# jcfaracco/xpysom-dask

Measured on AMD Instinct MI355X. Metric: samples/sec/epoch, higher is better.
Workload: dtype f16

## Files before the change

xpysom_dask_amd/_lib.py:

```python
import ctypes as C
import importlib.util
import os

HERE = os.path.dirname(os.path.abspath(__file__))
LIB_PATH = os.environ.get("SOM_LIB_PATH") or os.path.join(HERE, "libsomhip.so")

SOM_DIST = {"euclidean": 0, "euclidean_no_opt": 1, "cosine": 2, "manhattan": 3, "manhattan_no_opt": 3,
            "norm_p": 4, "norm_p_no_opt": 5}
SOM_NEIGH = {"gaussian": 0, "mexican_hat": 1, "bubble": 2, "triangle": 3}
SOM_PREC = {"f32": 0, "bf16": 1, "f16": 3, "exact": 5}
SOM_TOPO = {"rectangular": 0, "hexagonal": 1}
SOM_BMU_ACTIVATION, SOM_BMU_QUANTIZATION = 0, 1
SOM_KERNELS = {"bmu": 0, "segsum": 1, "kron": 2, "merge": 3, "prep": 4, "screen": 5}


class SomConfig(C.Structure):
    _fields_ = [("x", C.c_int32), ("y", C.c_int32), ("input_len", C.c_int32),
                ("distance", C.c_int32), ("neighborhood", C.c_int32),
                ("compact_support", C.c_int32), ("precision", C.c_int32), ("device", C.c_int32),
                ("std_coeff", C.c_double), ("stream", C.c_void_p),
                ("topology", C.c_int32), ("norm_p", C.c_int32), ("norm_p_real", C.c_double)]


_F = C.POINTER(C.c_float)
# ... 24 lines not shown
    "som_comm_init": (C.c_int, [_H, C.c_int32, C.c_int32, C.c_void_p]),
    "som_epoch_allreduce": (C.c_int, [_H]),
    "som_comm_destroy": (C.c_int, [_H]),
    "som_pinned_alloc": (C.c_int, [C.c_uint64, C.POINTER(C.c_void_p)]),
    "som_pinned_free": (C.c_int, [C.c_void_p]),
    "som_stream_begin": (C.c_int, [_H]),
    "som_stream_rows": (C.c_int, [_H, _F, C.c_int64]),
    "som_stream_end": (C.c_int, [_H, C.c_double, C.c_double, C.c_int]),
    "som_accum_device_ptr": (C.c_int, [_H, C.POINTER(C.c_void_p), C.POINTER(C.c_int64)]),
    "som_get_stream": (C.c_int, [_H, C.POINTER(C.c_void_p)]),
    "som_epoch_fetch": (C.c_int, [_H, _F, _F, _I]),
    "som_epoch_accumulate_forced": (C.c_int, [_H, _I, C.c_double, C.c_double, C.c_int]),
    "som_bmu": (C.c_int, [_H, _F, C.c_int64, C.c_int32, _I]),
    "som_bmu_device": (C.c_int, [_H, C.c_void_p, C.c_int64, C.c_int32, _I]),
    "som_bmu_top2": (C.c_int, [_H, _F, C.c_int64, _I, _I]),
    "som_bmu_top2_device": (C.c_int, [_H, C.c_void_p, C.c_int64, _I, _I]),
    "som_bmu_f64": (C.c_int, [_H, C.POINTER(C.c_double), C.c_int64, _I]),
    "som_distance_matrix": (C.c_int, [_H, _F, C.c_int64, C.c_int32, _F]),
    "som_quantization_error": (C.c_int, [_H, _F, C.c_int64, C.POINTER(C.c_double)]),
    "som_quantization_error_device": (C.c_int, [_H, C.c_void_p, C.c_int64, C.POINTER(C.c_double)]),
    "som_set_verify": (C.c_int, [_H, C.c_int32]),
    "som_verify_stats": (C.c_int, [_H, C.POINTER(C.c_int64), C.POINTER(C.c_int64)]),
    "som_debug_corrupt_operands": (C.c_int, [_H, C.c_int32]),
    "som_debug_mfma16": (C.c_int, [_H, C.c_void_p, C.c_void_p, _F, _F, C.c_int32]),
    "som_debug_stamps": (C.c_int, [_H, C.c_int64, C.c_void_p]),
    "som_debug_device_bytes": (C.c_int, [C.POINTER(C.c_int64)]),
    "som_debug_qe_stats": (C.c_int, [_H, C.POINTER(C.c_int64), C.POINTER(C.c_int64)]),
    "som_policy_eval": (C.c_int, [C.c_int32, C.POINTER(C.c_double), C.POINTER(C.c_double), C.POINTER(C.c_int32)]),
    "som_policy_replay": (C.c_int, [C.c_int32, C.POINTER(C.c_double), C.POINTER(C.c_double)]),
    "som_patch_order": (C.c_int, [C.c_int32, C.c_int32, _I]),
    "som_exact_stats": (C.c_int, [_H, C.POINTER(C.c_int64), C.POINTER(C.c_int64), C.POINTER(C.c_int64)]),
    "som_exact_top2_stats": (C.c_int, [_H, C.POINTER(C.c_int64), C.POINTER(C.c_int64)]),
    "som_exact_skip_stats": (C.c_int, [_H, C.POINTER(C.c_int64), C.POINTER(C.c_int64)]),
    "som_exact_resident_stats": (C.c_int, [_H, C.POINTER(C.c_int64), C.POINTER(C.c_int64)]),
    "som_exact_scout_stats": (C.c_int, [_H, C.POINTER(C.c_int64), C.POINTER(C.c_int64)]),
    "som_exact_refine_stats": (C.c_int, [_H, C.POINTER(C.c_int64), C.POINTER(C.c_int64)]),
    "som_exact_last_counts": (C.c_int, [_H, _I, C.c_int64]),
    "som_sync": (C.c_int, [_H]),
    "som_profile_enable": (C.c_int, [_H, C.c_int32]),
    "som_profile_get": (C.c_int, [_H, C.c_int32, C.POINTER(C.c_double), C.POINTER(C.c_int64)]),
    "som_profile_reset": (C.c_int, [_H]),
}

_lib = None


# ... 50 lines not shown
```

xpysom_dask_amd/csrc/bmu_bf16_k16.hpp:

```cpp
#pragma once
#include "bmu_bf16.hpp"

namespace somhip {

constexpr int K16_T = 4;
constexpr int K16_STAGE_UNITS = 16 * K16_T;
constexpr int K16_SB = 4;
constexpr int K16_NW = 4;
constexpr int K16_WG_SAMPLES = K16_NW * 16 * K16_SB;

__host__ __device__ constexpr int k16_stage_bytes(int ks32) { return (K16_T * ks32 + 1) * 1024; }

template <int KS32, class EL = Bf16>
__global__ __launch_bounds__(256) void prep_w_bf16_k16_kernel(const float* __restrict__ W, int K, int D,
                                                              char* __restrict__ Wst, int n_stages,
                                                              const float* __restrict__ unit_wsq,
                                                              const float* __restrict__ scale_max2 = nullptr) {
    using E = typename EL::T;
    using bf16x8 = typename V8<E>::t;
    long id = (long)blockIdx.x * 256 + threadIdx.x;
    long total = (long)n_stages * K16_T * KS32 * 64;
    if (id >= total) return;
    int lane = id & 63;
    long t = id >> 6;
    int ks = t % KS32; t /= KS32;
    int t16 = t % K16_T;
    long stage = t / K16_T;
    long u = stage * K16_STAGE_UNITS + t16 * 16 + (lane & 15);
    int k0 = ks * 32 + (lane >> 4) * 8;
    float scale = 1.0f;
    if (unit_wsq != nullptr && u < K) { float q = unit_wsq[u]; scale = q > 0.0f ? 1.0f / __builtin_sqrtf(q) : 0.0f; }
    if (scale_max2 != nullptr) scale = ex_scale(*scale_max2);
    bf16x8 v;
#pragma unroll
    for (int j = 0; j < 8; ++j) {
        float f = (u < K && k0 + j < D) ? W[u * D + k0 + j] * scale : 0.0f;
        v[j] = cvt<E>(-f);
    }
    *(bf16x8*)(Wst + stage * k16_stage_bytes(KS32) + ((long)(t16 * KS32 + ks) * 64 + lane) * 16) = v;
}

template <int KS32, class EL = Bf16>
__global__ __launch_bounds__(256) void prep_w_exact_k16_kernel(const float* __restrict__ W, int K, int D,
                                                               char* __restrict__ Wst, int n_stages,
                                                               const float* __restrict__ scale_max2,
                                                               float* __restrict__ werr2, char* __restrict__ Wst_lo = nullptr) {
    using E = typename EL::T;
    using bf16x8 = typename V8<E>::t;
    const int lane = threadIdx.x & 63;
    const long tile = (long)blockIdx.x * 4 + (threadIdx.x >> 6);
    if (tile >= (long)n_stages * K16_T) return;
    const long stage = tile / K16_T;
    const int t16 = (int)(tile - stage * K16_T);
    const long u = stage * K16_STAGE_UNITS + t16 * 16 + (lane & 15);
    const float scale = ex_scale(*scale_max2);
    float er = 0.0f;
#pragma unroll
    for (int ks = 0; ks < KS32; ++ks) {
        const int k0 = ks * 32 + (lane >> 4) * 8;
        bf16x8 v, vl;
#pragma unroll
        for (int j = 0; j < 8; ++j) {
            const float f = (u < K && k0 + j < D) ? W[u * D + k0 + j] * scale : 0.0f;
            const E hb = cvt<E>(-f);
            v[j] = hb;
            const float e = half_operand_error(-f, (float)hb);
            er = __builtin_fmaf(e, e, er);
            const float r = ((-f) - (float)hb) * 2048.0f;
            vl[j] = cvt<E>(r == r && __builtin_fabsf(r) < 3.0e38f ? r : 0.0f);
        }
        *(bf16x8*)(Wst + stage * k16_stage_bytes(KS32) + ((long)(t16 * KS32 + ks) * 64 + lane) * 16) = v;
        if (Wst_lo != nullptr) *(bf16x8*)(Wst_lo + stage * k16_stage_bytes(KS32) + ((long)(t16 * KS32 + ks) * 64 + lane) * 16) = vl;
// ... 417 lines not shown
```

xpysom_dask_amd/csrc/bmu_f32.hpp:

```cpp
#pragma once
#include "som_common.hpp"

namespace somhip {

constexpr int F32_SB = 128;
constexpr int F32_UB = 128;
constexpr int F32_KC = 32;

enum { SCORE_EUCLID_PART = 0, SCORE_EUCLID_SQRT = 1, SCORE_COSINE = 2, SCORE_EUCLID_SQ = 3 };

template <int MODE>
__device__ __forceinline__ float score_f32(float cross, float wsq, float xsq) {
    if (MODE == SCORE_EUCLID_PART) {
        return __builtin_fmaf(-2.0f, cross, wsq);
    } else if (MODE == SCORE_EUCLID_SQ) {
        return __builtin_fmaf(-2.0f, cross, wsq) + xsq;
    } else if (MODE == SCORE_EUCLID_SQRT) {
        float t = __builtin_fmaf(-2.0f, cross, wsq) + xsq;
        return nan_to_num_f32(__builtin_sqrtf(t));
    } else {
        float den = __builtin_sqrtf(xsq * wsq);
        return 1.0f - nan_to_num_f32(cross / den);
    }
}
// ... 76 lines not shown
        if (kc == 0 && tid < F32_UB) wq[tid] = (u0 + tid < K) ? wsq[u0 + tid] : 0.0f;
        __syncthreads();
        const float* xrow = Xs + (wave * 32 + col) * xstride + half;
        const float* wrow = Ws + col * (F32_KC + 1) + half;
#pragma unroll
        for (int k = 0; k < F32_KC; k += 2) {
            float b = xrow[k];
#pragma unroll
            for (int rb = 0; rb < 4; ++rb)
                acc[rb] = __builtin_amdgcn_mfma_f32_32x32x2f32(wrow[rb * 32 * (F32_KC + 1) + k], b, acc[rb], 0, 0, 0);
        }
    }
    if (my_sample < N) {
#pragma unroll
        for (int rb = 0; rb < 4; ++rb)
#pragma unroll
            for (int r = 0; r < 16; ++r) {
                int row = rb * 32 + mfma32_row(r, half);
                if (u0 + row < K) out[my_sample * K + u0 + row] = score_f32<MODE>(acc[rb][r], wq[row], xs);
            }
    }
}

__device__ float np_pairwise_sq_sum(const float* __restrict__ a, int n) {
    if (n < 8) {
        float res = 0.0f;
        for (int i = 0; i < n; ++i) res = __fadd_rn(res, __fmul_rn(a[i], a[i]));
        return res;
    }
    if (n <= 128) {
        float r[8];
#pragma unroll
        for (int j = 0; j < 8; ++j) r[j] = __fmul_rn(a[j], a[j]);
        int i = 8;
        for (; i < n - (n % 8); i += 8) {
#pragma unroll
            for (int j = 0; j < 8; ++j) r[j] = __fadd_rn(r[j], __fmul_rn(a[i + j], a[i + j]));
        }
        float res = __fadd_rn(__fadd_rn(__fadd_rn(r[0], r[1]), __fadd_rn(r[2], r[3])),
                              __fadd_rn(__fadd_rn(r[4], r[5]), __fadd_rn(r[6], r[7])));
        for (; i < n; ++i) res = __fadd_rn(res, __fmul_rn(a[i], a[i]));
        return res;
    }
    int n2 = n / 2;
    n2 -= n2 % 8;
    return __fadd_rn(np_pairwise_sq_sum(a, n2), np_pairwise_sq_sum(a + n2, n - n2));
}

__global__ __launch_bounds__(256) void row_sq_f32_kernel(const float* __restrict__ A, long rows, int D,
                                                         float* __restrict__ out, float* __restrict__ out_p = nullptr,
                                                         const int* __restrict__ inv = nullptr) {
    long row = (long)blockIdx.x * 256 + threadIdx.x;
    if (row >= rows) return;
    const float q = np_pairwise_sq_sum(A + row * (long)D, D);
    out[row] = q;
    if (out_p != nullptr) {
        out_p[inv[row]] = q;
    }
}

}
```

xpysom_dask_amd/csrc/exact_host.hpp:

```cpp

struct PassCtr {
    int* base; int n_groups;
    int* gcount() const { return base; }
    int* gstart() const { return base + n_groups; }
    PassCounters* tail() const { return (PassCounters*)(gstart() + n_groups); }
    RowNeed* row_need() const { return (RowNeed*)base; }
    size_t bytes() const { return 2 * (size_t)n_groups * sizeof(int) + sizeof(PassCounters); }
};
inline PassCtr pass_ctr(const som_handle* h) { return PassCtr{h->ex.ctr, (int)cdiv(h->K, EX_GROUP)}; }

constexpr double EX_KAPPA = 6.0;
ExactBound exact_bound(const som_handle* h) {
    const double u = std::ldexp(1.0, -24);
    const double Dl = h->wide ? 32.0 * h->ft_kchunks : 8.0 * h->fr_kg;
    const double n_mfma = h->wide ? h->n_kchunks : h->ks32;
    const double gamma = Dl * u / (1.0 - Dl * u);
    const double slop = 1.01;
    ExactBound eb{};
    eb.cB = (float)(slop * 2.0 * (EX_KAPPA * n_mfma + 1.0) * std::ldexp(1.0, -23));
    eb.cM = (float)(slop * 2.0);
    if (h->cfg.distance == SOM_DIST_COSINE) {
        eb.cA = (float)(slop * 2.0 * (gamma + 57.0 * u));
        eb.cW = 0.0f;
        eb.unit = 1;
// ... 244 lines not shown
        if (int rc = ex.tq.alloc(h, (size_t)stride)) return rc;
    if (int rc = ex.need.alloc(h, (size_t)tiles * ex.cen[0].n_cstages)) return rc;
    if (int rc = ex.need2.alloc(h, (size_t)tiles * ex.cen[1].n_cstages)) return rc;
    if (int rc = ex.glist.alloc(h, (size_t)tiles * n_groups)) return rc;
    if (int rc = ex.gcnt.alloc(h, (size_t)tiles)) return rc;
    if (int rc = ex.tile_counts.alloc(h, (size_t)tiles)) return rc;
    if (int rc = ex.tlist.alloc(h, (size_t)tiles * n_groups * K16_T)) return rc;
    if (int rc = ex.tcnt.alloc(h, (size_t)tiles)) return rc;
    ex.item_slots = (int)resident_slots(h, 8);
    if (int rc = ex.items.alloc(h, (size_t)(5 * tiles + 4 * ex.item_slots + 16))) return rc;
    if (int rc = ex.sk_tmp.alloc(h, radix_scratch_ints(stride))) return rc;
    ex.sk_stride = stride;
    return 0;
}

template <class E>
int exact_skip_centroids(som_handle* h, const float* xmax2) {
    auto& ex = h->ex;
    const float* Wsrc = h->ex_patch ? h->Wp : h->W;
    const int n_groups = (int)cdiv(h->K, EX_GROUP);
    auto& c0 = ex.cen[0];
    auto& c1 = ex.cen[1];
    const CentroidLevel l1{c0.Cc, c0.rg, c0.csq, c0.cmax2, c0.n_slots}, l2{c1.Cc, c1.rg, c1.csq, c1.cmax2, c1.n_slots};
    exact_centroids_kernel<<<dim3((unsigned)(cdiv(n_groups, 4) * 4)), dim3(512), 0, h->stream>>>(Wsrc, h->K, h->D, n_groups, l1, l2, h->wmax2);
    const int nst2 = ex.lp.level2 ? c1.n_cstages : 0;
    char* plain = ex.lp.scout ? c0.Cst_plain : nullptr;
    const dim3 tgrid((unsigned)cdiv((long)(c0.n_cstages + nst2) * K16_T, 4)), block(256);
    switch (h->ks32) {
#define SOM_CIMG_CASE(k) case k: exact_centroid_image_kernel<k, E><<<tgrid, block, 0, h->stream>>>(l1, c0.Cst, c0.n_cstages, l2, c1.Cst, nst2, h->D, xmax2, h->wmax2, plain); break;
    SOM_CIMG_CASE(1) SOM_CIMG_CASE(2) SOM_CIMG_CASE(3) SOM_CIMG_CASE(4)
#undef SOM_CIMG_CASE
    default: return fail(h, "exact: block skipping supports input_len <= 128");
    }
    HIPCHK(h, hipGetLastError());
    return 0;
}

int exact_skip_sortkeys(som_handle* h, som_handle::ExactScratch::SortedRows& sr, long s0, long n, const int* prev, const int* scout_g) {
    auto& ex = h->ex;
    const int n_groups = (int)cdiv(h->K, EX_GROUP);
    if (scout_g != nullptr)
        exact_groupkey_kernel<<<dim3((unsigned)cdiv(n, 256)), dim3(256), 0, h->stream>>>(scout_g, n, n_groups, ex.sk_keys, ex.sk_vals);
    else
        exact_sortkey_kernel<<<dim3((unsigned)cdiv(n, 256)), dim3(256), 0, h->stream>>>(prev, h->ex_inv, n, h->K, ex.sk_keys, ex.sk_vals);
    int bits = 1;
    while ((1L << bits) < n_groups) ++bits;
    return radix_sort_rows(h, ex.sk_keys, n, bits, ex.sk_keys2, sr.order + s0, ex.sk_tmp);
// ... 597 lines not shown
```

xpysom_dask_amd/csrc/exact_skip.hpp:

```cpp
#pragma once
#include "bmu_bf16_k16.hpp"

namespace somhip {

constexpr int SK_TILE = K16_WG_SAMPLES;
static_assert(K16_STAGE_UNITS == 64 && K16_T == 4, "block skipping: a stage of the resident screen is one 64-unit group of four 16-unit tiles");

struct CentroidLevel { float* C; float* rg; float* csq; float* cmax2; int n_slots; };
__global__ __launch_bounds__(512) void exact_centroids_kernel(const float* __restrict__ W, int K, int D, int n_groups,
                                                              CentroidLevel l1, CentroidLevel l2, const float* __restrict__ wmax2) {
    __shared__ float qsum[4][128];
    __shared__ float part[2][64][2];
    __shared__ float csq_s[2][5];
    const int g = blockIdx.x, tid = threadIdx.x, lane = tid & 63;
    const int d = tid & 127, q = tid >> 7, fh = (tid >> 6) & 1;
    const long u0 = (long)g * 64 + 16 * q;
    const int cnt = (int)max(0L, min(64L, (long)K - (long)g * 64));
    const int cb = max(0, min(16, cnt - 16 * q));
    if (g == 0 && tid == 0) { l1.cmax2[0] = *wmax2; l1.cmax2[1] = 0.0f; l2.cmax2[0] = *wmax2; l2.cmax2[1] = 0.0f; }
    float w[16];
#pragma unroll
    for (int k = 0; k < 16; ++k) w[k] = (d < D && k < cb) ? W[(u0 + k) * D + d] : 0.0f;
    float sum = 0.0f;
#pragma unroll
    for (int k = 0; k < 16; ++k) sum += w[k];
    qsum[q][d] = sum;
    __syncthreads();
    const float cs = cb > 0 ? sum / (float)cb : 0.0f;
    const float cg = cnt > 0 ? ((qsum[0][d] + qsum[1][d]) + (qsum[2][d] + qsum[3][d])) / (float)cnt : 0.0f;
    if (d < D) {
        if (q == 0 && g < l1.n_slots) l1.C[(long)g * D + d] = cg;
        const int j = 16 * (g >> 2) + 4 * (g & 3) + q;
        if (j < l2.n_slots) l2.C[(long)j * D + d] = cs;
    }
    {
        const float a = wave_sum(cs * cs);
        if (lane == 0) csq_s[fh][1 + q] = a;
        if (q == 0) { const float bq = wave_sum(cg * cg); if (lane == 0) csq_s[fh][0] = bq; }
    }
#pragma unroll
    for (int k = 0; k < 16; ++k) {
        if (k < cb) {
            const float dg = w[k] - cg, ds = w[k] - cs;
            const float qg = wave_sum(d < D ? dg * dg : 0.0f);
            const float qs = wave_sum(d < D ? ds * ds : 0.0f);
            if (lane == 0) { part[fh][16 * q + k][0] = qg; part[fh][16 * q + k][1] = qs; }
        }
    }
    __syncthreads();
    if (tid < 5) {
        const int b = tid - 1;
        const int k0 = tid == 0 ? 0 : 16 * b, k1 = tid == 0 ? cnt : min(cnt, 16 * b + 16);
        float m = 0.0f;
        for (int k = k0; k < k1; ++k) {
            const float d2 = part[0][k][tid == 0 ? 0 : 1] + part[1][k][tid == 0 ? 0 : 1];
            m = (d2 > m || !(d2 == d2)) ? d2 : m;
        }
        const float r = k1 > k0 ? __builtin_sqrtf(m) * (1.0f + 1.0f / 512.0f) + 1.0e-30f : -1.0f;
        const float sq = csq_s[0][tid] + csq_s[1][tid];
        if (tid == 0) { if (g < l1.n_slots) { l1.rg[g] = r; l1.csq[g] = sq; } }
        else {
            const int j = 16 * (g >> 2) + 4 * (g & 3) + b;
            if (j < l2.n_slots) { l2.rg[j] = r; l2.csq[j] = sq; }
        }
    }
}

__global__ __launch_bounds__(256) void exact_sortkey_kernel(const int* __restrict__ prev, const int* __restrict__ inv, long n,
                                                            int K, int* __restrict__ keys, int* __restrict__ vals) {
    const long i = (long)blockIdx.x * 256 + threadIdx.x;
    if (i >= n) return;
    int u = prev[i];
    u = u < 0 ? 0 : u >= K ? K - 1 : u;
    keys[i] = (inv != nullptr ? inv[u] : u) >> 6;
    vals[i] = (int)i;
}

__global__ __launch_bounds__(256) void exact_lastpos_kernel(const int* __restrict__ prev, const int* __restrict__ order,
                                                            const int* __restrict__ inv, long n, int K, int* __restrict__ lastpos) {
    const long p = (long)blockIdx.x * 256 + threadIdx.x;
    if (p >= n) return;
    int u = prev[order[p]];
    u = u < 0 ? 0 : u >= K ? K - 1 : u;
    lastpos[p] = inv != nullptr ? inv[u] : u;
}

template <class EL>
// ... 648 lines not shown
```

xpysom_dask_amd/csrc/somhip.hip:

```cpp
#include <hip/hip_runtime.h>

#include <cstring>

#include <dlfcn.h>

#include <cmath>
#include <cstdio>
#include <cstdlib>
#include <algorithm>
#include <atomic>
#include <cstring>
#include <string>
#include <utility>
#include <vector>

#include "../../include/somhip.h"
#include "../../include/somhip_test.h"
#include "bmu_bf16_k16.hpp"
#include "bmu_bf16_tiled.hpp"
#include "bmu_bf16_wide.hpp"
#include "bmu_exact.hpp"
#include "exact_skip.hpp"
#include "exact_policy.hpp"
#include "exact_skip_wide.hpp"
// ... 88 lines not shown
        DevBuf<float> fbX;
        PassCounters* pass_host = nullptr;
        hipEvent_t fb_ready = nullptr;
        int64_t rows_total = 0, rows_fallback = 0, chunks = 0;
        int64_t blocks_run = 0, blocks_total = 0;
        long pass_rows_override = 0;
        long hook_refuse_above = 0, hook_pairs = 0; bool hook_refuse_skip = false;
        long stride_cap = 0;
        long pairs = 64;
        int skip_mode = 1;
        policy::PlanState plan;
        policy::LaunchPlan lp;
        bool sub_blocks = true;
        struct SortedRows {
            long cap = 0;
            DevBuf<int> order;
            DevBuf<__bf16> Xb_s;
            DevBuf<__bf16> Xl_s;
            bool xl_filled = false;
            DevBuf<float> Xf_s, xsq_s, xerr_s, seed_s, sU_s;
            DevBuf<int> lastpos_s;
        } srt[2];
        bool cen_ready = false;
        long sk_stride = 0;
        int res_every = 0;
        DevBuf<int> sk_keys, sk_keys2, sk_vals;
        DevBuf<int> sk_tmp;
        bool refine_on = true;
        int grid_mult = 2;
        bool scout_on = true;
        DevBuf<int> scout_g;
        DevBuf<float> tq;
        double share_forecast = 1.0;
        struct Cost {
            hipEvent_t ev[8] = {};
            bool have = false;
        } cost;
        struct Centroids { DevBuf<float> Cc, rg, csq, cmax2; DevBuf<char> Cst;
                           DevBuf<char> Cst_plain;
                           int n_slots = 0, n_cstages = 0, n_img_stages = 0; } cen[2];
        DevBuf<unsigned long long> need, need2;
        DevBuf<int> glist, gcnt;
        DevBuf<int> tlist, tcnt;
        DevBuf<int2> tile_counts;
        DevBuf<int2> items;
        int item_slots = 0;
// ... 7 lines not shown
    bool wide = false;
    int tl_bm = 128, tl_bn = 128, tl_xtile = 0, tl_wfrag = 0, tl_wtile = 0;
    int dp = 0;
    int stage_bytes = 0;
    int stage_units = 0;
    int nt = 1;
    bool swapped = false;
    int norm_p = 2;
    double norm_pr = 0.0;
    hipStream_t stream = nullptr;
    bool own_stream = false;

    DevBuf<float> W, wsq, SC, T, ACC, P1, P2;
    DevBuf<float> Ud;
    DevBuf<char> Wst;
    DevBuf<char> Wst_lo;
    DevBuf<char> Wfst;
    int fr_kg = 0, fr_stages = 0;
    DevBuf<char> Wfimg;
    DevBuf<char> ftX;
    int ft_kchunks = 0, ft_ublocks = 0;
    int n_stages = 0;
    bool w_dirty = true, wsq_dirty = true, wf_dirty = true, wp_dirty = true;

    const float* Xd = nullptr;
    DevBuf<float> X_owned;
    long N = 0, Np = 0;
    DevBuf<int> bmu;
    bool bmu_valid = false;
    struct EarlyUpdate { bool armed = false, done = false; double sigma = 0, eta = 0; int neigh_f64 = 0; } early;
    DevBuf<unsigned long long> best64;
    int n_cus = 0;
    struct SegScratch {
        DevBuf<int> skey, srow;
        DevBuf<int> tmp;
        DevBuf<int> kA, kB;
        DevBuf<float> vA, vB;
        long cap = 0;
        DevBuf<int> cs_table;
        long cs_blocks = 0;
    };
    SegScratch seg;
    DevBuf<float> xsq;
    DevBuf<__bf16> Xb;
    DevBuf<float> xmax2;
    DevBuf<float> wn;
// ... 164 lines not shown
        float ms = 0.f;
        HIPCHK(h, hipEventElapsedTime(&ms, ep.a, ep.b));
        h->ms[ep.kernel] += ms;
        h->launches[ep.kernel] += 1;
        h->pool.push_back(ep);
    }
    h->pending.clear();
    return 0;
}

#define SOM_HALF(h, fn, ...) ((h)->f16 ? fn<F16>(__VA_ARGS__) : fn<Bf16>(__VA_ARGS__))
#define SOM_KS32_DISPATCH(fn, ...) \
    switch (h->ks32) { \
    case 1: return fn<1, E>(__VA_ARGS__); case 2: return fn<2, E>(__VA_ARGS__); case 3: return fn<3, E>(__VA_ARGS__); case 4: return fn<4, E>(__VA_ARGS__); }
#define SOM_WIDE_DISPATCH(fn, ...) \
    switch (h->n_kchunks) { \
    case 5: return fn<5, E>(__VA_ARGS__); case 6: return fn<6, E>(__VA_ARGS__); case 7: return fn<7, E>(__VA_ARGS__); case 8: return fn<8, E>(__VA_ARGS__); \
    case 9: return fn<9, E>(__VA_ARGS__); case 10: return fn<10, E>(__VA_ARGS__); case 11: return fn<11, E>(__VA_ARGS__); case 12: return fn<12, E>(__VA_ARGS__); \
    case 13: return fn<13, E>(__VA_ARGS__); case 14: return fn<14, E>(__VA_ARGS__); case 15: return fn<15, E>(__VA_ARGS__); case 16: return fn<16, E>(__VA_ARGS__); \
    case 17: return fn<17, E>(__VA_ARGS__); case 18: return fn<18, E>(__VA_ARGS__); case 19: return fn<19, E>(__VA_ARGS__); case 20: return fn<20, E>(__VA_ARGS__); \
    case 21: return fn<21, E>(__VA_ARGS__); case 22: return fn<22, E>(__VA_ARGS__); case 23: return fn<23, E>(__VA_ARGS__); case 24: return fn<24, E>(__VA_ARGS__); \
    case 25: return fn<25, E>(__VA_ARGS__); }

void mark_codebook_changed(som_handle* h) { h->w_dirty = h->wsq_dirty = h->wf_dirty = h->wp_dirty = true; }

template <class E>
int prep_codebook_half(som_handle* h) {
    const float* unit = h->cfg.distance == SOM_DIST_COSINE ? h->wsq : nullptr;
    const float* Wex = h->ex_patch ? h->Wp : h->W;
    const float* qex = h->ex_patch ? h->wsq_p : h->wsq;
    const dim3 block(256);
    if (h->tiled) {
        if (h->wide && h->exact) {
            if (unit) unit = qex;
            if (unit) {
                HIPCHK(h, hipMemsetAsync(h->wn, 0, (size_t)h->K * sizeof(float), h->stream));
                HIPCHK(h, hipMemsetD32Async((hipDeviceptr_t)h->wmax2, 0x3F800000, 1, h->stream));
            } else {
                HIPCHK(h, hipMemsetAsync(h->wmax2, 0, sizeof(float), h->stream));
                exact_copy_wsq_kernel<<<dim3((unsigned)cdiv(h->K, 1024)), dim3(1024), 0, h->stream>>>(qex, h->K, h->wn, h->wmax2);
            }
            long total = (long)h->n_stages * WD_T * h->n_kchunks * 64;
            prep_w_bf16_wide_kernel<E><<<dim3((unsigned)cdiv(total, 256)), block, 0, h->stream>>>(
                Wex, h->K, h->D, h->n_kchunks, h->Wst, h->n_stages, unit, h->wmax2);
            HIPCHK(h, hipMemsetAsync(h->wmax2 + 1, 0, sizeof(float), h->stream));
            exact_werr_kernel<E><<<dim3((unsigned)cdiv(h->K, 4 * EX_WERR_UNITS)), block, 0, h->stream>>>(Wex, h->K, h->D, h->wmax2, h->wmax2 + 1, unit);
            return 0;
        }
        if (h->wide) {
            long total = (long)h->n_stages * WD_T * h->n_kchunks * 64;
            prep_w_bf16_wide_kernel<E><<<dim3((unsigned)cdiv(total, 256)), block, 0, h->stream>>>(
                h->W, h->K, h->D, h->n_kchunks, h->Wst, h->n_stages, unit);
        } else {
            long total = (long)h->n_ublocks * h->n_kchunks * (h->tl_bn / 16) * TL_KS * 64;
            prep_tiles_bf16_kernel<E><<<dim3((unsigned)cdiv(total, 256)), block, 0, h->stream>>>(
                h->W, h->K, h->D, h->n_kchunks, h->n_ublocks, h->tl_bn, h->tl_wtile, -1.0f, unit, h->Wst);
        }
        HIPCHK(h, hipMemsetAsync(h->wmax2, 0, sizeof(float), h->stream));
        rownorm_bf16_kernel<E><<<dim3((unsigned)cdiv(h->K, 4)), block, 0, h->stream>>>(
            h->W, h->K, h->D, unit, unit != nullptr, h->wn, h->wmax2);
        return 0;
    }
    const long total = (long)h->n_stages * K16_T * h->ks32 * 64;
    const dim3 grid((unsigned)cdiv(total, 256));
    if (h->exact) {
        HIPCHK(h, hipMemsetAsync(h->wmax2, 0, 2 * sizeof(float), h->stream));
        exact_copy_wsq_kernel<<<dim3((unsigned)cdiv(h->K, 1024)), dim3(1024), 0, h->stream>>>(qex, h->K, h->wn, h->wmax2);
        const dim3 tgrid((unsigned)cdiv((long)h->n_stages * K16_T, 4));
        switch (h->ks32) {
        case 1: prep_w_exact_k16_kernel<1, E><<<tgrid, block, 0, h->stream>>>(Wex, h->K, h->D, h->Wst, h->n_stages, h->wmax2, h->wmax2 + 1, h->Wst_lo); break;
        case 2: prep_w_exact_k16_kernel<2, E><<<tgrid, block, 0, h->stream>>>(Wex, h->K, h->D, h->Wst, h->n_stages, h->wmax2, h->wmax2 + 1, h->Wst_lo); break;
        case 3: prep_w_exact_k16_kernel<3, E><<<tgrid, block, 0, h->stream>>>(Wex, h->K, h->D, h->Wst, h->n_stages, h->wmax2, h->wmax2 + 1, h->Wst_lo); break;
        case 4: prep_w_exact_k16_kernel<4, E><<<tgrid, block, 0, h->stream>>>(Wex, h->K, h->D, h->Wst, h->n_stages, h->wmax2, h->wmax2 + 1, h->Wst_lo); break;
        default: return fail(h, "the resident half-precision kernel supports input_len <= 128");
        }
        return 0;
    }
    const float* sc = nullptr;
    switch (h->ks32) {
    case 1: prep_w_bf16_k16_kernel<1, E><<<grid, block, 0, h->stream>>>(h->W, h->K, h->D, h->Wst, h->n_stages, unit, sc); break;
    case 2: prep_w_bf16_k16_kernel<2, E><<<grid, block, 0, h->stream>>>(h->W, h->K, h->D, h->Wst, h->n_stages, unit, sc); break;
    case 3: prep_w_bf16_k16_kernel<3, E><<<grid, block, 0, h->stream>>>(h->W, h->K, h->D, h->Wst, h->n_stages, unit, sc); break;
    case 4: prep_w_bf16_k16_kernel<4, E><<<grid, block, 0, h->stream>>>(h->W, h->K, h->D, h->Wst, h->n_stages, unit, sc); break;
    default: return fail(h, "the resident half-precision kernel supports input_len <= 128");
    }
    HIPCHK(h, hipMemsetAsync(h->wmax2, 0, sizeof(float), h->stream));
    prep_wnorm_kernel<E><<<dim3((unsigned)cdiv(h->K, 256)), block, 0, h->stream>>>(h->W, h->K, h->D, h->wn, h->wmax2, unit);
    return 0;
}

int refresh_codebook_operands(som_handle* h, bool need_f32, bool patch = false) {
    if (h->exact) need_f32 = true;
    patch = patch && h->ex_patch;
    const bool bf = h->cfg.precision != SOM_PREC_F32;
    const bool do_f32 = (need_f32 || !bf) && (h->wf_dirty || h->wf_patch != patch);
    const bool do_bf = bf && h->w_dirty;
// ... 1176 lines not shown
    if (!out) return 1;
    *out = nullptr;
    if (hipHostMalloc(out, bytes ? bytes : 1, hipHostMallocDefault) != hipSuccess) { (void)hipGetLastError(); return 1; }
    return 0;
}

int som_pinned_free(void* p) {
    if (p && hipHostFree(p) != hipSuccess) { (void)hipGetLastError(); return 1; }
    return 0;
}

int som_stream_end(som_handle* h, double sigma, double eta, int neigh_f64) {
    DeviceGuard dev_guard(h);
    if (!h) return 1;
    if (!h->streaming) return fail(h, "som_stream_end: call som_stream_begin first");
    h->streaming = false;
    return run_transform(h, sigma, eta, neigh_f64);
}

int som_epoch_merge(som_handle* h) {
    DeviceGuard dev_guard(h);
    if (!h) return 1;
    Timed t(h, SOM_K_MERGE);
    if (h->fuse_merge_prep && ((is_half1(h) && !h->tiled && h->cfg.distance == SOM_DIST_EUCLIDEAN) ||
                               (h->wide && !h->exact && h->n_kchunks <= 4 * WD_MP_ITERS))) {
        if (int rc = SOM_HALF(h, merge_prep_half, h)) return rc;
        HIPCHK(h, hipGetLastError());
        mark_codebook_changed(h);
        h->w_dirty = false;
        return 0;
    }
    long total = (long)h->K * h->D;
    const bool keep_wp = h->ex_patch && !h->wp_dirty;
    merge_kernel<<<dim3((unsigned)cdiv(total, 256)), dim3(256), 0, h->stream>>>(h->W, h->ACC, h->K, h->D, h->D1p,
                                                                                keep_wp ? h->Wp : nullptr, h->ex_inv);
    HIPCHK(h, hipGetLastError());
    mark_codebook_changed(h);
    if (keep_wp) h->wp_dirty = false;
    return 0;
}

int som_epoch_accumulate_begin(som_handle* h, double sigma, double eta, int neigh_f64);
int som_epoch_accumulate_block(som_handle* h, int32_t block, int64_t* offset, int64_t* n_floats);

namespace {
int rccl_load(const char* path) {
// ... 363 lines not shown
}

int som_verify_stats(som_handle* h, int64_t* launches, int64_t* rows_checked) {
    if (!h) return 1;
    if (launches) *launches = h->verify_launches;
    if (rows_checked) *rows_checked = h->verify_rows_checked;
    return 0;
}

int som_debug_corrupt_operands(som_handle* h, int32_t which) {
    DeviceGuard dev_guard(h);
    if (!h) return 1;
    if (int rc = refresh_codebook_operands(h, true, h->exact)) return rc;
    if ((which & 1) && h->Wst) {
        size_t bytes = (size_t)h->n_stages * h->stage_bytes;
        if (h->tiled && !h->wide) bytes = (size_t)h->n_ublocks * h->n_kchunks * h->tl_wtile;
        HIPCHK(h, hipMemsetAsync(h->Wst, 0, bytes, h->stream));
    }
    if ((which & 2) && h->Wfst) HIPCHK(h, hipMemsetAsync(h->Wfst, 0, (size_t)h->fr_stages * fr_stage_bytes(h->fr_kg), h->stream));
    if ((which & 2) && h->Wfimg) HIPCHK(h, hipMemsetAsync(h->Wfimg, 0, (size_t)h->ft_ublocks * h->ft_kchunks * FT_WTILE, h->stream));
    return 0;
}

int som_policy_eval(int32_t which, const double* costs, const double* args, int32_t* out) {
    if (!costs || !args || !out) return 1;
    policy::Costs c;
    c.full_total = costs[0]; c.full_screen = costs[1]; c.plan_total = costs[2]; c.plan_over = costs[3]; c.plan_over_scout = costs[4];
    c.blk_ms = costs[5]; c.l2_ms_group = costs[6]; c.l2_ratio = costs[7]; c.sort_ms = costs[8];
    switch (which) {
    case 0: *out = policy::commit_scouted_plan(c, args[0], args[1]); return 0;
    case 1: *out = policy::level2_from_sample(c, args[0], args[1], args[2]); return 0;
    case 2: *out = policy::level2_pays(c, args[0], args[1]); return 0;
    case 3: *out = policy::sort_paid(c, args[0], args[1], args[2], (int)args[3]); return 0;
    case 4: *out = policy::plan_idle(c, args[0]); return 0;
    case 5: *out = policy::scout_continues(c, args[0], args[1], args[2]); return 0;
    case 6: *out = policy::rows_worth_a_scout(args[0], args[1], args[2]); return 0;
    }
    return 1;
}

int som_policy_replay(int32_t n_launches, const double* script, double* out) {
    if (n_launches < 0 || !script || !out) return 1;
    policy::PlanState st;
    for (int32_t i = 0; i < n_launches; ++i) {
        const double* in = script + (size_t)i * SOM_POLICY_REPLAY_IN;
        double* o = out + (size_t)i * SOM_POLICY_REPLAY_OUT;
// ... 169 lines not shown
```

Measured before the change: 504.6 million.

## Fuse exact-mode merge with codebook prep and centroid computation

Adds a fused kernel for exact, non-tiled mode. In one pass over each 64-unit group it normalises the accumulators into the codebook, writes the permuted copy, squared norms, float32 stage image and max norm, and rebuilds the centroid levels. Freshness flags let the later prep skip its separate norm-copy and centroid kernels and reset the centroid max inside the exact prep kernel. This cuts kernel launches and repeated passes over the codebook, at the cost of more complex state tracking. A debug CRC entry point is also added.

```diff
diff --git a/xpysom_dask_amd/_lib.py b/xpysom_dask_amd/_lib.py
--- a/xpysom_dask_amd/_lib.py
+++ b/xpysom_dask_amd/_lib.py
@@ -70,6 +70,7 @@
     "som_set_verify": (C.c_int, [_H, C.c_int32]),
     "som_verify_stats": (C.c_int, [_H, C.POINTER(C.c_int64), C.POINTER(C.c_int64)]),
     "som_debug_corrupt_operands": (C.c_int, [_H, C.c_int32]),
+    "som_debug_operand_crc": (C.c_int, [_H, C.c_int32, C.POINTER(C.c_uint64)]),
     "som_debug_mfma16": (C.c_int, [_H, C.c_void_p, C.c_void_p, _F, _F, C.c_int32]),
     "som_debug_stamps": (C.c_int, [_H, C.c_int64, C.c_void_p]),
     "som_debug_device_bytes": (C.c_int, [C.POINTER(C.c_int64)]),
diff --git a/xpysom_dask_amd/csrc/bmu_bf16_k16.hpp b/xpysom_dask_amd/csrc/bmu_bf16_k16.hpp
--- a/xpysom_dask_amd/csrc/bmu_bf16_k16.hpp
+++ b/xpysom_dask_amd/csrc/bmu_bf16_k16.hpp
@@ -44,10 +44,12 @@
 __global__ __launch_bounds__(256) void prep_w_exact_k16_kernel(const float* __restrict__ W, int K, int D,
                                                                char* __restrict__ Wst, int n_stages,
                                                                const float* __restrict__ scale_max2,
-                                                               float* __restrict__ werr2, char* __restrict__ Wst_lo = nullptr) {
+                                                               float* __restrict__ werr2, char* __restrict__ Wst_lo = nullptr,
+                                                               float* __restrict__ cm1 = nullptr, float* __restrict__ cm2 = nullptr) {
     using E = typename EL::T;
     using bf16x8 = typename V8<E>::t;
     const int lane = threadIdx.x & 63;
+    if (cm1 != nullptr && blockIdx.x == 0 && threadIdx.x == 0) { cm1[0] = *scale_max2; cm1[1] = 0.0f; cm2[0] = *scale_max2; cm2[1] = 0.0f; }
     const long tile = (long)blockIdx.x * 4 + (threadIdx.x >> 6);
     if (tile >= (long)n_stages * K16_T) return;
     const long stage = tile / K16_T;
diff --git a/xpysom_dask_amd/csrc/bmu_f32.hpp b/xpysom_dask_amd/csrc/bmu_f32.hpp
--- a/xpysom_dask_amd/csrc/bmu_f32.hpp
+++ b/xpysom_dask_amd/csrc/bmu_f32.hpp
@@ -122,26 +122,28 @@
     }
 }
 
-__device__ float np_pairwise_sq_sum(const float* __restrict__ a, int n) {
+template <class P>
+__device__ __forceinline__ float np_pairwise_sq_sum_leaf(P a, int n) {
     if (n < 8) {
         float res = 0.0f;
         for (int i = 0; i < n; ++i) res = __fadd_rn(res, __fmul_rn(a[i], a[i]));
         return res;
     }
-    if (n <= 128) {
-        float r[8];
+    float r[8];
 #pragma unroll
-        for (int j = 0; j < 8; ++j) r[j] = __fmul_rn(a[j], a[j]);
-        int i = 8;
-        for (; i < n - (n % 8); i += 8) {
+    for (int j = 0; j < 8; ++j) r[j] = __fmul_rn(a[j], a[j]);
+    int i = 8;
+    for (; i < n - (n % 8); i += 8) {
 #pragma unroll
-            for (int j = 0; j < 8; ++j) r[j] = __fadd_rn(r[j], __fmul_rn(a[i + j], a[i + j]));
-        }
-        float res = __fadd_rn(__fadd_rn(__fadd_rn(r[0], r[1]), __fadd_rn(r[2], r[3])),
-                              __fadd_rn(__fadd_rn(r[4], r[5]), __fadd_rn(r[6], r[7])));
-        for (; i < n; ++i) res = __fadd_rn(res, __fmul_rn(a[i], a[i]));
-        return res;
+        for (int j = 0; j < 8; ++j) r[j] = __fadd_rn(r[j], __fmul_rn(a[i + j], a[i + j]));
     }
+    float res = __fadd_rn(__fadd_rn(__fadd_rn(r[0], r[1]), __fadd_rn(r[2], r[3])),
+                          __fadd_rn(__fadd_rn(r[4], r[5]), __fadd_rn(r[6], r[7])));
+    for (; i < n; ++i) res = __fadd_rn(res, __fmul_rn(a[i], a[i]));
+    return res;
+}
+__device__ float np_pairwise_sq_sum(const float* __restrict__ a, int n) {
+    if (n <= 128) return np_pairwise_sq_sum_leaf(a, n);
     int n2 = n / 2;
     n2 -= n2 % 8;
     return __fadd_rn(np_pairwise_sq_sum(a, n2), np_pairwise_sq_sum(a + n2, n - n2));
diff --git a/xpysom_dask_amd/csrc/exact_host.hpp b/xpysom_dask_amd/csrc/exact_host.hpp
--- a/xpysom_dask_amd/csrc/exact_host.hpp
+++ b/xpysom_dask_amd/csrc/exact_host.hpp
@@ -290,7 +290,8 @@
     auto& c0 = ex.cen[0];
     auto& c1 = ex.cen[1];
     const CentroidLevel l1{c0.Cc, c0.rg, c0.csq, c0.cmax2, c0.n_slots}, l2{c1.Cc, c1.rg, c1.csq, c1.cmax2, c1.n_slots};
-    exact_centroids_kernel<<<dim3((unsigned)(cdiv(n_groups, 4) * 4)), dim3(512), 0, h->stream>>>(Wsrc, h->K, h->D, n_groups, l1, l2, h->wmax2);
+    if (!ex.cen_fresh)
+        exact_centroids_kernel<<<dim3((unsigned)(cdiv(n_groups, 4) * 4)), dim3(512), 0, h->stream>>>(Wsrc, h->K, h->D, n_groups, l1, l2, h->wmax2);
     const int nst2 = ex.lp.level2 ? c1.n_cstages : 0;
     char* plain = ex.lp.scout ? c0.Cst_plain : nullptr;
     const dim3 tgrid((unsigned)cdiv((long)(c0.n_cstages + nst2) * K16_T, 4)), block(256);
diff --git a/xpysom_dask_amd/csrc/exact_skip.hpp b/xpysom_dask_amd/csrc/exact_skip.hpp
--- a/xpysom_dask_amd/csrc/exact_skip.hpp
+++ b/xpysom_dask_amd/csrc/exact_skip.hpp
@@ -1,5 +1,6 @@
 #pragma once
 #include "bmu_bf16_k16.hpp"
+#include "bmu_f32_res.hpp"
 
 namespace somhip {
 
@@ -7,13 +8,67 @@
 static_assert(K16_STAGE_UNITS == 64 && K16_T == 4, "block skipping: a stage of the resident screen is one 64-unit group of four 16-unit tiles");
 
 struct CentroidLevel { float* C; float* rg; float* csq; float* cmax2; int n_slots; };
+struct CentroidShared {
+    float qsum[4][128];
+    float part[2][64][2];
+    float csq_s[2][5];
+};
+__device__ __forceinline__ void group_centroids(const float (&w)[16], int g, int K, int D, const CentroidLevel& l1,
+                                                const CentroidLevel& l2, CentroidShared& sh) {
+    const int tid = threadIdx.x, lane = tid & 63;
+    const int d = tid & 127, q = tid >> 7, fh = (tid >> 6) & 1;
+    const int cnt = (int)max(0L, min(64L, (long)K - (long)g * 64));
+    const int cb = max(0, min(16, cnt - 16 * q));
+    float sum = 0.0f;
+#pragma unroll
+    for (int k = 0; k < 16; ++k) sum += w[k];
+    sh.qsum[q][d] = sum;
+    __syncthreads();
+    const float cs = cb > 0 ? sum / (float)cb : 0.0f;
+    const float cg = cnt > 0 ? ((sh.qsum[0][d] + sh.qsum[1][d]) + (sh.qsum[2][d] + sh.qsum[3][d])) / (float)cnt : 0.0f;
+    if (d < D) {
+        if (q == 0 && g < l1.n_slots) l1.C[(long)g * D + d] = cg;
+        const int j = 16 * (g >> 2) + 4 * (g & 3) + q;
+        if (j < l2.n_slots) l2.C[(long)j * D + d] = cs;
+    }
+    {
+        const float a = wave_sum(cs * cs);
+        if (lane == 0) sh.csq_s[fh][1 + q] = a;
+        if (q == 0) { const float bq = wave_sum(cg * cg); if (lane == 0) sh.csq_s[fh][0] = bq; }
+    }
+#pragma unroll
+    for (int k = 0; k < 16; ++k) {
+        if (k < cb) {
+            const float dg = w[k] - cg, ds = w[k] - cs;
+            const float qg = wave_sum(d < D ? dg * dg : 0.0f);
+            const float qs = wave_sum(d < D ? ds * ds : 0.0f);
+            if (lane == 0) { sh.part[fh][16 * q + k][0] = qg; sh.part[fh][16 * q + k][1] = qs; }
+        }
+    }
+    __syncthreads();
+    if (tid < 5) {
+        const int b = tid - 1;
+        const int k0 = tid == 0 ? 0 : 16 * b, k1 = tid == 0 ? cnt : min(cnt, 16 * b + 16);
+        float m = 0.0f;
+        for (int k = k0; k < k1; ++k) {
+            const float d2 = sh.part[0][k][tid == 0 ? 0 : 1] + sh.part[1][k][tid == 0 ? 0 : 1];
+            m = (d2 > m || !(d2 == d2)) ? d2 : m;
+        }
+        const float r = k1 > k0 ? __builtin_sqrtf(m) * (1.0f + 1.0f / 512.0f) + 1.0e-30f : -1.0f;
+        const float sq = sh.csq_s[0][tid] + sh.csq_s[1][tid];
+        if (tid == 0) { if (g < l1.n_slots) { l1.rg[g] = r; l1.csq[g] = sq; } }
+        else {
+            const int j = 16 * (g >> 2) + 4 * (g & 3) + b;
+            if (j < l2.n_slots) { l2.rg[j] = r; l2.csq[j] = sq; }
+        }
+    }
+}
+
 __global__ __launch_bounds__(512) void exact_centroids_kernel(const float* __restrict__ W, int K, int D, int n_groups,
                                                               CentroidLevel l1, CentroidLevel l2, const float* __restrict__ wmax2) {
-    __shared__ float qsum[4][128];
-    __shared__ float part[2][64][2];
-    __shared__ float csq_s[2][5];
-    const int g = blockIdx.x, tid = threadIdx.x, lane = tid & 63;
-    const int d = tid & 127, q = tid >> 7, fh = (tid >> 6) & 1;
+    __shared__ CentroidShared sh;
+    const int g = blockIdx.x, tid = threadIdx.x;
+    const int d = tid & 127, q = tid >> 7;
     const long u0 = (long)g * 64 + 16 * q;
     const int cnt = (int)max(0L, min(64L, (long)K - (long)g * 64));
     const int cb = max(0, min(16, cnt - 16 * q));
@@ -21,48 +76,87 @@
     float w[16];
 #pragma unroll
     for (int k = 0; k < 16; ++k) w[k] = (d < D && k < cb) ? W[(u0 + k) * D + d] : 0.0f;
-    float sum = 0.0f;
-#pragma unroll
-    for (int k = 0; k < 16; ++k) sum += w[k];
-    qsum[q][d] = sum;
-    __syncthreads();
-    const float cs = cb > 0 ? sum / (float)cb : 0.0f;
-    const float cg = cnt > 0 ? ((qsum[0][d] + qsum[1][d]) + (qsum[2][d] + qsum[3][d])) / (float)cnt : 0.0f;
-    if (d < D) {
-        if (q == 0 && g < l1.n_slots) l1.C[(long)g * D + d] = cg;
-        const int j = 16 * (g >> 2) + 4 * (g & 3) + q;
-        if (j < l2.n_slots) l2.C[(long)j * D + d] = cs;
-    }
-    {
-        const float a = wave_sum(cs * cs);
-        if (lane == 0) csq_s[fh][1 + q] = a;
-        if (q == 0) { const float bq = wave_sum(cg * cg); if (lane == 0) csq_s[fh][0] = bq; }
-    }
+    group_centroids(w, g, K, D, l1, l2, sh);
+}
+
+constexpr int MPX_STRIDE = 129;
+static_assert(FR_STAGE_UNITS == 64, "the fused merge writes one float32 stage per 64-unit group");
+struct MergePrepOut {
+    float* W; float* Wp; const int* perm;
+    float* wsq; float* wsq_p; float* wn; float* wmax2;
+    char* Wfst; int fr_kg;
+};
+__global__ __launch_bounds__(512) void exact_merge_prep_kernel(const float* __restrict__ ACC, int K, int D, int D1p, int n_groups,
+                                                               MergePrepOut o, CentroidLevel l1, CentroidLevel l2) {
+    __shared__ CentroidShared sh;
+    __shared__ float ws[64 * MPX_STRIDE];
+    __shared__ int u_s[64];
+    __shared__ float den_s[64];
+    const int g = blockIdx.x, tid = threadIdx.x;
+    const int d = tid & 127, q = tid >> 7;
+    const int cnt = (int)max(0L, min(64L, (long)K - (long)g * 64));
+    const int cb = max(0, min(16, cnt - 16 * q));
+    if (tid < cnt) {
+        const int pos = g * 64 + tid;
+        const int u = o.perm != nullptr ? o.perm[pos] : pos;
+        u_s[tid] = u;
+        den_s[tid] = ACC[(long)u * D1p + D];
+    }
+    __syncthreads();
+    float w[16];
 #pragma unroll
     for (int k = 0; k < 16; ++k) {
-        if (k < cb) {
-            const float dg = w[k] - cg, ds = w[k] - cs;
-            const float qg = wave_sum(d < D ? dg * dg : 0.0f);
-            const float qs = wave_sum(d < D ? ds * ds : 0.0f);
-            if (lane == 0) { part[fh][16 * q + k][0] = qg; part[fh][16 * q + k][1] = qs; }
-        }
-    }
-    __syncthreads();
-    if (tid < 5) {
-        const int b = tid - 1;
-        const int k0 = tid == 0 ? 0 : 16 * b, k1 = tid == 0 ? cnt : min(cnt, 16 * b + 16);
-        float m = 0.0f;
-        for (int k = k0; k < k1; ++k) {
-            const float d2 = part[0][k][tid == 0 ? 0 : 1] + part[1][k][tid == 0 ? 0 : 1];
-            m = (d2 > m || !(d2 == d2)) ? d2 : m;
-        }
-        const float r = k1 > k0 ? __builtin_sqrtf(m) * (1.0f + 1.0f / 512.0f) + 1.0e-30f : -1.0f;
-        const float sq = csq_s[0][tid] + csq_s[1][tid];
-        if (tid == 0) { if (g < l1.n_slots) { l1.rg[g] = r; l1.csq[g] = sq; } }
-        else {
-            const int j = 16 * (g >> 2) + 4 * (g & 3) + b;
-            if (j < l2.n_slots) { l2.rg[j] = r; l2.csq[j] = sq; }
-        }
+        const bool on = d < D && k < cb;
+        const long u = on ? u_s[16 * q + k] : 0;
+        const float* src = !on ? ACC : den_s[16 * q + k] != 0.0f ? ACC + u * D1p + d : o.W + u * D + d;
+        const float v = *src;
+        w[k] = on ? v : 0.0f;
+    }
+#pragma unroll
+    for (int k = 0; k < 16; ++k) {
+        const bool on = d < D && k < cb;
+        const int i = 16 * q + k;
+        const float den = on ? den_s[i] : 0.0f;
+        const float v = w[k] / den;
+        w[k] = den != 0.0f ? v : w[k];
+        if (on) {
+            const long u = u_s[i];
+            if (den != 0.0f) o.W[u * D + d] = w[k];
+            if (o.Wp != nullptr) o.Wp[((long)g * 64 + i) * D + d] = w[k];
+            ws[i * MPX_STRIDE + d] = w[k];
+        }
+    }
+    if (l1.C != nullptr) group_centroids(w, g, K, D, l1, l2, sh);
+    else __syncthreads();
+    if (g >= n_groups) return;
+    if (o.Wfst != nullptr) {
+        char* base = o.Wfst + (long)g * fr_stage_bytes(o.fr_kg);
+        for (int r = tid; r < FR_UT * o.fr_kg * 64; r += 512) {
+            const int lane = r & 63, t = r >> 6;
+            const int gk = t % o.fr_kg, i = (t / o.fr_kg) * 32 + (lane & 31);
+            f32x4 v;
+#pragma unroll
+            for (int j = 0; j < 4; ++j) {
+                const int k = 8 * gk + 2 * j + (lane >> 5);
+                v[j] = (i < cnt && k < D) ? ws[i * MPX_STRIDE + k] : 0.0f;
+            }
+            *(f32x4*)(base + (long)r * 16) = v;
+        }
+    }
+    if (tid < 64) {
+        float qv = __builtin_inff(), m = 0.0f;
+        if (tid < cnt) {
+            const int pos = g * 64 + tid;
+            qv = np_pairwise_sq_sum_leaf((const float*)(ws + tid * MPX_STRIDE), D);
+            o.wsq[u_s[tid]] = qv;
+            if (o.wsq_p != nullptr) o.wsq_p[pos] = qv;
+            o.wn[pos] = qv;
+            m = (qv == qv) ? qv : 0.0f;
+        }
+        if (o.Wfst != nullptr) ((float*)(o.Wfst + (long)g * fr_stage_bytes(o.fr_kg) + (long)FR_UT * o.fr_kg * 1024))[tid] = qv;
+#pragma unroll
+        for (int s = 32; s > 0; s >>= 1) m = fmaxf(m, __shfl_xor(m, s, 64));
+        if (tid == 0) atomic_max_pos_f32(o.wmax2, m);
     }
 }
 
diff --git a/xpysom_dask_amd/csrc/somhip.hip b/xpysom_dask_amd/csrc/somhip.hip
--- a/xpysom_dask_amd/csrc/somhip.hip
+++ b/xpysom_dask_amd/csrc/somhip.hip
@@ -134,6 +134,7 @@
             DevBuf<int> lastpos_s;
         } srt[2];
         bool cen_ready = false;
+        bool cen_fresh = false;
         long sk_stride = 0;
         int res_every = 0;
         DevBuf<int> sk_keys, sk_keys2, sk_vals;
@@ -187,6 +188,7 @@
     int ft_kchunks = 0, ft_ublocks = 0;
     int n_stages = 0;
     bool w_dirty = true, wsq_dirty = true, wf_dirty = true, wp_dirty = true;
+    bool wn_fresh = false;
 
     const float* Xd = nullptr;
     DevBuf<float> X_owned;
@@ -397,7 +399,10 @@
     case 21: return fn<21, E>(__VA_ARGS__); case 22: return fn<22, E>(__VA_ARGS__); case 23: return fn<23, E>(__VA_ARGS__); case 24: return fn<24, E>(__VA_ARGS__); \
     case 25: return fn<25, E>(__VA_ARGS__); }
 
-void mark_codebook_changed(som_handle* h) { h->w_dirty = h->wsq_dirty = h->wf_dirty = h->wp_dirty = true; }
+void mark_codebook_changed(som_handle* h) {
+    h->w_dirty = h->wsq_dirty = h->wf_dirty = h->wp_dirty = true;
+    h->wn_fresh = false; h->ex.cen_fresh = false;
+}
 
 template <class E>
 int prep_codebook_half(som_handle* h) {
@@ -439,14 +444,18 @@
     const long total = (long)h->n_stages * K16_T * h->ks32 * 64;
     const dim3 grid((unsigned)cdiv(total, 256));
     if (h->exact) {
-        HIPCHK(h, hipMemsetAsync(h->wmax2, 0, 2 * sizeof(float), h->stream));
-        exact_copy_wsq_kernel<<<dim3((unsigned)cdiv(h->K, 1024)), dim3(1024), 0, h->stream>>>(qex, h->K, h->wn, h->wmax2);
+        if (!h->wn_fresh) {
+            HIPCHK(h, hipMemsetAsync(h->wmax2, 0, 2 * sizeof(float), h->stream));
+            exact_copy_wsq_kernel<<<dim3((unsigned)cdiv(h->K, 1024)), dim3(1024), 0, h->stream>>>(qex, h->K, h->wn, h->wmax2);
+        }
+        h->wn_fresh = false;
+        float* cm1 = h->ex.cen_fresh ? (float*)h->ex.cen[0].cmax2 : nullptr;
+        float* cm2 = h->ex.cen_fresh ? (float*)h->ex.cen[1].cmax2 : nullptr;
         const dim3 tgrid((unsigned)cdiv((long)h->n_stages * K16_T, 4));
         switch (h->ks32) {
-        case 1: prep_w_exact_k16_kernel<1, E><<<tgrid, block, 0, h->stream>>>(Wex, h->K, h->D, h->Wst, h->n_stages, h->wmax2, h->wmax2 + 1, h->Wst_lo); break;
-        case 2: prep_w_exact_k16_kernel<2, E><<<tgrid, block, 0, h->stream>>>(Wex, h->K, h->D, h->Wst, h->n_stages, h->wmax2, h->wmax2 + 1, h->Wst_lo); break;
-        case 3: prep_w_exact_k16_kernel<3, E><<<tgrid, block, 0, h->stream>>>(Wex, h->K, h->D, h->Wst, h->n_stages, h->wmax2, h->wmax2 + 1, h->Wst_lo); break;
-        case 4: prep_w_exact_k16_kernel<4, E><<<tgrid, block, 0, h->stream>>>(Wex, h->K, h->D, h->Wst, h->n_stages, h->wmax2, h->wmax2 + 1, h->Wst_lo); break;
+#define SOM_PREPX_CASE(k) case k: prep_w_exact_k16_kernel<k, E><<<tgrid, block, 0, h->stream>>>(Wex, h->K, h->D, h->Wst, h->n_stages, h->wmax2, h->wmax2 + 1, h->Wst_lo, cm1, cm2); break;
+        SOM_PREPX_CASE(1) SOM_PREPX_CASE(2) SOM_PREPX_CASE(3) SOM_PREPX_CASE(4)
+#undef SOM_PREPX_CASE
         default: return fail(h, "the resident half-precision kernel supports input_len <= 128");
         }
         return 0;
@@ -1669,6 +1678,29 @@
     DeviceGuard dev_guard(h);
     if (!h) return 1;
     Timed t(h, SOM_K_MERGE);
+    if (h->fuse_merge_prep && h->exact && !h->tiled) {
+        const int n_groups = (int)cdiv(h->K, EX_GROUP);
+        const bool cen = h->ex.cen_ready;
+        HIPCHK(h, hipMemsetAsync(h->wmax2, 0, 2 * sizeof(float), h->stream));
+        const MergePrepOut o{h->W, h->ex_patch ? (float*)h->Wp : nullptr, h->ex_patch ? (const int*)h->ex_perm : nullptr,
+                             h->wsq, h->ex_patch ? (float*)h->wsq_p : nullptr, h->wn, h->wmax2, h->Wfst, h->fr_kg};
+        CentroidLevel l1{nullptr, nullptr, nullptr, nullptr, 0}, l2 = l1;
+        if (cen) {
+            auto& c0 = h->ex.cen[0];
+            auto& c1 = h->ex.cen[1];
+            l1 = CentroidLevel{c0.Cc, c0.rg, c0.csq, c0.cmax2, c0.n_slots};
+            l2 = CentroidLevel{c1.Cc, c1.rg, c1.csq, c1.cmax2, c1.n_slots};
+        }
+        const unsigned grid = (unsigned)(cen ? cdiv(n_groups, 4) * 4 : n_groups);
+        exact_merge_prep_kernel<<<dim3(grid), dim3(512), 0, h->stream>>>(h->ACC, h->K, h->D, h->D1p, n_groups, o, l1, l2);
+        HIPCHK(h, hipGetLastError());
+        mark_codebook_changed(h);
+        h->wsq_dirty = false; h->wp_dirty = false;
+        if (h->Wfst) { h->wf_dirty = false; h->wf_patch = h->ex_patch; }
+        h->wn_fresh = true;
+        h->ex.cen_fresh = cen;
+        return 0;
+    }
     if (h->fuse_merge_prep && ((is_half1(h) && !h->tiled && h->cfg.distance == SOM_DIST_EUCLIDEAN) ||
                                (h->wide && !h->exact && h->n_kchunks <= 4 * WD_MP_ITERS))) {
         if (int rc = SOM_HALF(h, merge_prep_half, h)) return rc;
@@ -2078,6 +2110,51 @@
     return 0;
 }
 
+int som_debug_operand_crc(som_handle* h, int32_t which, uint64_t* out) {
+    DeviceGuard dev_guard(h);
+    if (!h || !out) return 1;
+    uint64_t hash = 0xcbf29ce484222325ull;
+    std::vector<unsigned char> host;
+    auto add = [&](const void* dev, size_t bytes) -> int {
+        if (dev == nullptr || bytes == 0) return 0;
+        host.resize(bytes);
+        if (int rc = d2h_blocking(h, host.data(), dev, bytes)) return rc;
+        for (size_t i = 0; i < bytes; ++i) { hash ^= host[i]; hash *= 0x100000001b3ull; }
+        return 0;
+    };
+    HIPCHK(h, hipStreamSynchronize(h->stream));
+    const bool half = h->cfg.precision != SOM_PREC_F32;
+    size_t st_bytes = (size_t)h->n_stages * h->stage_bytes;
+    if (h->tiled && !h->wide) st_bytes = (size_t)h->n_ublocks * h->n_kchunks * h->tl_wtile;
+    int rc = 0;
+    switch (which) {
+    case 0: rc = add(h->Wst, half ? st_bytes : 0); break;
+    case 1: rc = add(h->Wst_lo, st_bytes); break;
+    case 2:
+        for (int st = 0; h->Wfst && st < h->fr_stages && rc == 0; ++st)
+            rc = add((const char*)h->Wfst + (size_t)st * fr_stage_bytes(h->fr_kg), (size_t)FR_UT * h->fr_kg * 1024 + 64 * sizeof(float));
+        break;
+    case 3: rc = add(h->ex_patch ? (const float*)h->wsq_p : (const float*)h->wsq, (size_t)h->K * sizeof(float)); break;
+    case 4: rc = add(h->wn, half ? (size_t)h->K * sizeof(float) : 0); break;
+    case 5: rc = add(h->wmax2, half ? 2 * sizeof(float) : 0); break;
+    case 6:
+        if (h->ex.cen_ready)
+            for (int lv = 0; lv < (h->wide ? 1 : 2) && rc == 0; ++lv) {
+                auto& c = h->ex.cen[lv];
+                if ((rc = add(c.Cc, (size_t)c.n_slots * h->D * sizeof(float)))) break;
+                if ((rc = add(c.rg, (size_t)c.n_slots * sizeof(float)))) break;
+                if ((rc = add(c.csq, (size_t)c.n_slots * sizeof(float)))) break;
+                rc = add(c.cmax2, 2 * sizeof(float));
+            }
+        break;
+    case 7: rc = add(h->ex_patch ? (const float*)h->Wp : (const float*)h->W, (size_t)h->K * h->D * sizeof(float)); break;
+    default: return fail(h, "som_debug_operand_crc: unknown buffer");
+    }
+    if (rc) return rc;
+    *out = hash;
+    return 0;
+}
+
 int som_policy_eval(int32_t which, const double* costs, const double* args, int32_t* out) {
     if (!costs || !args || !out) return 1;
     policy::Costs c;
```

Measured after the change: 513.7 million (median of 6 runs). +1.8%, better.
